# OPPO-Mente-Lab/X2I

Measured on AMD Instinct MI355X. Metric: images/sec, FLUX-schnell 1024x1024 4-step (projector + denoise loop), whole job, higher is better.
Workload: dtype bf16; 1 GPU; BASELINE configs[1]: qwen3b conditioning (C=37,H=2048,S_txt=512) -> projector -> shuttle-3/FLUX-schnell DiT 1024x1024, 4 steps; batch_per_gpu=4, global_batch=4, parallelism=batch-sharded x1, graph=True

## Files before the change

### x2i_amd/csrc/elementwise.hip

```cpp
#include "x2i_common.h"
#include "x2i_kernels.h"

namespace {

__device__ __forceinline__ void unpack8(const bf16x8_t& v, float (&f)[8]) {
#pragma unroll
  for (int i = 0; i < 8; ++i) f[i] = bf16_to_f32((bf16_t)v[i]);
}
__device__ __forceinline__ bf16x8_t pack8(const float (&f)[8]) {
  union { bf16x8_t v; uint32_t u[4]; } r;
#pragma unroll
  for (int i = 0; i < 4; ++i) r.u[i] = pack_bf16x2(f[2 * i], f[2 * i + 1]);
  return r.v;
}

constexpr int LN_MAXV = 8;

template <bool AFFINE>
__global__ __launch_bounds__(256) void ln_kernel(const bf16_t* __restrict__ X, long long x_bs, int ldx, bf16_t* __restrict__ Y,
                                                 long long y_bs, int ldy, int S, int D, int S0, const float* shift0,
                                                 const float* scale0, const float* shift1, const float* scale1,
                                                 long long mod_bs, const bf16_t* aw, const bf16_t* ab, float eps,
                                                 long long total_rows) {
  const int lane = threadIdx.x & 63;
// ... 193 lines not shown
                                                            int K, int act_in, int act_out, int accumulate, int rpw, long long x_gs, int rows_g) {
  typedef float f32x2 __attribute__((ext_vector_type(2)));
  if (blockIdx.y) {
    const long long g = blockIdx.y;
    Xv = (const char*)Xv + g * x_gs * (x_is_bf16 ? 2 : 4);
    W += g * N * K;
    if (bias) bias += g * N;
    Y += g * rows_g * ldy;
  }
  constexpr int NBP = NB == 1 ? 1 : (NB + 1) & ~1;
  extern __shared__ __attribute__((aligned(16))) float xs[];
  for (int i = threadIdx.x; i < NB * K; i += 256) {
    const int b = i / K, k = i - b * K;
    float v = x_is_bf16 ? bf16_to_f32(((const bf16_t*)Xv)[i]) : ((const float*)Xv)[i];
    xs[k * NBP + b] = apply_act(v, act_in);
  }
  __syncthreads();
  const int lane = threadIdx.x & 63;
  const int wave = threadIdx.x >> 6;
  const int n_base = (blockIdx.x * 4 + wave) * rpw;
  constexpr int R = 4;
  constexpr int NP = NB / 2;
#pragma unroll 1
  for (int rr = 0; rr < rpw; rr += R) {
    const int n0 = n_base + rr;
    if (n0 >= N) break;
    float acc[R][NB];
    f32x2 acc2[R][NP > 0 ? NP : 1];
#pragma unroll
    for (int r = 0; r < R; ++r) {
#pragma unroll
      for (int b = 0; b < NB; ++b) acc[r][b] = 0.f;
#pragma unroll
      for (int q = 0; q < NP; ++q) acc2[r][q] = f32x2{0.f, 0.f};
    }
    for (int k = lane * 8; k < K; k += 512) {
      bf16x8_t wv[R];
#pragma unroll
      for (int r = 0; r < R; ++r) {
        const int n = min(n0 + r, N - 1);
        wv[r] = __builtin_nontemporal_load((const bf16x8_t*)(W + (long long)n * K + k));
      }
      float wf[R][8];
#pragma unroll
      for (int r = 0; r < R; ++r) unpack8(wv[r], wf[r]);
#pragma unroll
      for (int j = 0; j < 8; ++j) {
        const float* xk = xs + (k + j) * NBP;
#pragma unroll
        for (int q = 0; q < NP; ++q) {
          const f32x2 x2 = *(const f32x2*)(xk + 2 * q);
#pragma unroll
          for (int r = 0; r < R; ++r) acc2[r][q] = __builtin_elementwise_fma(f32x2{wf[r][j], wf[r][j]}, x2, acc2[r][q]);
        }
        if constexpr (NB & 1) {
          const float x1 = xk[NB - 1];
#pragma unroll
          for (int r = 0; r < R; ++r) acc[r][NB - 1] = fmaf(wf[r][j], x1, acc[r][NB - 1]);
        }
      }
    }
#pragma unroll
    for (int r = 0; r < R; ++r)
#pragma unroll
      for (int q = 0; q < NP; ++q) { acc[r][2 * q] = acc2[r][q][0]; acc[r][2 * q + 1] = acc2[r][q][1]; }
#pragma unroll
    for (int r = 0; r < R; ++r) {
#pragma unroll
      for (int b = 0; b < NB; ++b) acc[r][b] = wave_sum(acc[r][b]);
      const int n = n0 + r;
      if (lane == 0 && n < N && rr + r < rpw) {
        const float bv = bias ? bf16_to_f32(bias[n]) : 0.f;
#pragma unroll
        for (int b = 0; b < NB; ++b) {
          float v = apply_act(acc[r][b] + bv, act_out);
          float* yp = Y + (long long)b * ldy + n;
          *yp = accumulate ? (*yp + v) : v;
        }
      }
    }
  }
}

__global__ void sinusoid_kernel(const float* __restrict__ t, float* __restrict__ out, int B, int dim, int round_bf16) {
  const int i = blockIdx.x * blockDim.x + threadIdx.x;
  const int half = dim / 2;
  if (i >= B * dim) return;
  const int b = i / dim, j = i - b * dim;
  const int k = j < half ? j : j - half;
  const float f = expf(-logf(10000.f) * (float)k / (float)half);
  const float a = t[b] * f;
  float v = j < half ? cosf(a) : sinf(a);
  if (round_bf16) v = bf16_to_f32(f32_to_bf16(v));
  out[i] = v;
}

__global__ void rope_table_kernel(const float* __restrict__ ids, int S, int d0, int d1, int d2, double theta, float* __restrict__ cosp,
                                  float* __restrict__ sinp) {
  const int D = d0 + d1 + d2;
  const long long i = (long long)blockIdx.x * blockDim.x + threadIdx.x;
  if (i >= (long long)S * D) return;
  const int s = (int)(i / D), c = (int)(i - (long long)s * D);
  int a = 0, start = 0, d = d0;
  if (c >= d0 + d1) a = 2, start = d0 + d1, d = d2;
  else if (c >= d0) a = 1, start = d0, d = d1;
  const int k = (c - start) >> 1;
  const double freq = 1.0 / pow(theta, (double)(2 * k) / (double)d);
  const double ang = (double)ids[(long long)s * 3 + a] * freq;
  cosp[i] = (float)cos(ang);
  sinp[i] = (float)sin(ang);
}

__global__ void euler_kernel(bf16_t* __restrict__ x, const bf16_t* __restrict__ eps, long long n8, const float* __restrict__ dt) {
  const float d = dt[0];
  for (long long i = (long long)blockIdx.x * blockDim.x + threadIdx.x; i < n8; i += (long long)gridDim.x * blockDim.x) {
    float a[8], e[8];
    unpack8(*(const bf16x8_t*)(x + i * 8), a);
    unpack8(*(const bf16x8_t*)(eps + i * 8), e);
#pragma unroll
    for (int j = 0; j < 8; ++j) a[j] = a[j] + d * e[j];
    *(bf16x8_t*)(x + i * 8) = pack8(a);
  }
}

__global__ __launch_bounds__(256) void gated_residual_kernel(bf16_t* __restrict__ X, long long x_bs, int ldx, const bf16_t* __restrict__ T,
                                                             long long t_bs, int ldt, const float* __restrict__ gate, long long g_bs, int S,
                                                             int D8, long long total) {
  for (long long i = (long long)blockIdx.x * blockDim.x + threadIdx.x; i < total; i += (long long)gridDim.x * blockDim.x) {
    const int c = (int)(i % D8);
    const long long row = i / D8;
    const int b = (int)(row / S), s = (int)(row - (long long)b * S);
    bf16_t* x = X + (long long)b * x_bs + (long long)s * ldx + c * 8;
    float a[8], t[8];
    unpack8(*(const bf16x8_t*)x, a);
    unpack8(*(const bf16x8_t*)(T + (long long)b * t_bs + (long long)s * ldt + c * 8), t);
    const float* g = gate + (long long)b * g_bs + c * 8;
#pragma unroll
    for (int j = 0; j < 8; ++j) a[j] = fmaf(g[j], t[j], a[j]);
    *(bf16x8_t*)x = pack8(a);
  }
}

__global__ void euler_tail_kernel(bf16_t* x, const bf16_t* eps, long long start, long long n, const float* dt) {
  const long long i = start + blockIdx.x * blockDim.x + threadIdx.x;
  if (i < n) x[i] = f32_to_bf16(bf16_to_f32(x[i]) + dt[0] * bf16_to_f32(eps[i]));
}

__global__ void cast_f32_bf16_kernel(const float* __restrict__ x, bf16_t* __restrict__ y, long long n) {
  for (long long i = (long long)blockIdx.x * blockDim.x + threadIdx.x; i < n; i += (long long)gridDim.x * blockDim.x)
    y[i] = f32_to_bf16(x[i]);
}
__global__ void cast_bf16_f32_kernel(const bf16_t* __restrict__ x, float* __restrict__ y, long long n) {
  for (long long i = (long long)blockIdx.x * blockDim.x + threadIdx.x; i < n; i += (long long)gridDim.x * blockDim.x)
    y[i] = bf16_to_f32(x[i]);
}

__global__ void seq_mean_kernel(const float* __restrict__ x, float* __restrict__ y, int S, int N) {
  const int n = blockIdx.x * blockDim.x + threadIdx.x, b = blockIdx.y;
  if (n >= N) return;
  const float* p = x + (long long)b * S * N + n;
  float acc = 0.f;
  for (int s = 0; s < S; ++s) acc += p[(long long)s * N];
  y[(long long)b * N + n] = acc / (float)S;
}

inline bool al16(const void* p) { return (((uintptr_t)p) & 15) == 0; }

}

int x2i_launch_ln_modulate(const void* X, long long x_bs, int ldx, void* Y, long long y_bs, int ldy, int B, int S, int D,
                           int S0, const float* shift0, const float* scale0, const float* shift1, const float* scale1,
                           long long mod_bs, float eps, hipStream_t stream) {
  if (!X || !Y || !shift1 || !scale1 || (S0 > 0 && (!shift0 || !scale0))) return x2i_set_error(X2I_ERR_ARG, "ln_modulate: null pointer");
  if (D % 8 || D > 64 * 8 * LN_MAXV || B <= 0 || S <= 0) return x2i_set_error(X2I_ERR_SHAPE, "ln_modulate: D=%d must be a multiple of 8 and <= %d", D, 64 * 8 * LN_MAXV);
  if (ldx % 8 || ldy % 8 || x_bs % 8 || y_bs % 8 || mod_bs % 4 || !al16(X) || !al16(Y)) return x2i_set_error(X2I_ERR_ALIGN, "ln_modulate: rows must be 16-byte aligned");
  const long long rows = (long long)B * S;
  if (D == 3072 && rows >= 4096) {
    hipLaunchKernelGGL((ln_rows_kernel<6, 4>), dim3((unsigned)((rows + 15) / 16)), dim3(256), 0, stream, (const bf16_t*)X, x_bs, ldx, (bf16_t*)Y, y_bs,
                       ldy, S, S0, shift0 ? shift0 : shift1, scale0 ? scale0 : scale1, shift1, scale1, mod_bs, eps, rows);
    return x2i_check_launch("ln_modulate");
  }
  hipLaunchKernelGGL(ln_kernel<false>, dim3((unsigned)((rows + 3) / 4)), dim3(256), 0, stream, (const bf16_t*)X, x_bs, ldx,
                     (bf16_t*)Y, y_bs, ldy, S, D, S0, shift0 ? shift0 : shift1, scale0 ? scale0 : scale1, shift1, scale1, mod_bs,
                     (const bf16_t*)nullptr, (const bf16_t*)nullptr, eps, rows);
  return x2i_check_launch("ln_modulate");
}

int x2i_launch_ln_affine(const void* X, void* Y, long long rows, int D, const void* w, const void* b, float eps, hipStream_t stream) {
  if (!X || !Y || !w || !b) return x2i_set_error(X2I_ERR_ARG, "ln_affine: null pointer");
  if (D % 8 || D > 64 * 8 * LN_MAXV || rows <= 0) return x2i_set_error(X2I_ERR_SHAPE, "ln_affine: D=%d unsupported", D);
  if (!al16(X) || !al16(Y) || !al16(w) || !al16(b)) return x2i_set_error(X2I_ERR_ALIGN, "ln_affine: 16-byte alignment required");
  hipLaunchKernelGGL(ln_kernel<true>, dim3((unsigned)((rows + 3) / 4)), dim3(256), 0, stream, (const bf16_t*)X, (long long)0, D,
                     (bf16_t*)Y, (long long)0, D, (int)1 << 30, D, 0, (const float*)nullptr, (const float*)nullptr,
                     (const float*)nullptr, (const float*)nullptr, (long long)0, (const bf16_t*)w, (const bf16_t*)b, eps, rows);
  return x2i_check_launch("ln_affine");
}

int x2i_launch_qkv_split(const void* qkv0, const void* qkv1, int ld0, int ld1, int B, int S, int S0, int H, const void* nq0,
                         const void* nk0, const void* nq1, const void* nk1, const float* cosp, const float* sinp, void* Q,
                         void* K, void* VT, int Spad, float eps, hipStream_t stream) {
  if (S0 < 0 || S0 > S || B <= 0 || S <= 0 || H <= 0) return x2i_set_error(X2I_ERR_SHAPE, "qkv_split: bad shape");
  if ((S0 > 0 && (!qkv0 || !nq0 || !nk0)) || (S0 < S && (!qkv1 || !nq1 || !nk1)) || !cosp || !sinp || !Q || !K || !VT)
    return x2i_set_error(X2I_ERR_ARG, "qkv_split: null pointer");
  if (Spad % 128 || Spad < S) return x2i_set_error(X2I_ERR_SHAPE, "qkv_split: Spad=%d must be a multiple of 128 and >= S=%d", Spad, S);
  if ((S0 > 0 && ld0 % 8) || (S0 < S && ld1 % 8)) return x2i_set_error(X2I_ERR_ALIGN, "qkv_split: ld must be a multiple of 8");
  hipLaunchKernelGGL(qk_norm_rope_kernel, dim3(S, B), dim3(256), 0, stream, (const bf16_t*)qkv0, (const bf16_t*)qkv1, ld0, ld1, S,
                     S0, H, (const bf16_t*)nq0, (const bf16_t*)nk0, (const bf16_t*)nq1, (const bf16_t*)nk1, cosp, sinp, (bf16_t*)Q,
                     (bf16_t*)K, Spad, eps);
  int rc = x2i_check_launch("qk_norm_rope");
  if (rc) return rc;
  hipLaunchKernelGGL(v_transpose_kernel, dim3((S + 63) / 64, H, B), dim3(256), 0, stream, (const bf16_t*)qkv0, (const bf16_t*)qkv1,
                     ld0, ld1, S, S0, H, (bf16_t*)VT, Spad);
  return x2i_check_launch("v_transpose");
}

int x2i_launch_skinny_linear(const void* X, int x_is_bf16, const void* W, const void* bias, float* Y, int ldy, int B, int N, int K,
                             int act_in, int act_out, int accumulate, hipStream_t stream) {
  return x2i_launch_skinny_linear_grouped(X, x_is_bf16, 0, W, bias, Y, ldy, 1, B, N, K, act_in, act_out, accumulate, stream);
}

int x2i_launch_skinny_linear_grouped(const void* X, int x_is_bf16, long long x_gs, const void* W, const void* bias, float* Y, int ldy, int G, int B,
                                     int N, int K, int act_in, int act_out, int accumulate, hipStream_t stream) {
  if (!X || !W || !Y) return x2i_set_error(X2I_ERR_ARG, "skinny_linear: null pointer");
  if (G <= 0 || G > 65535 || x_gs < 0) return x2i_set_error(X2I_ERR_SHAPE, "skinny_linear: bad group count / stride (G=%d)", G);
  if (G > 1 && B > SK_MAXB) return x2i_set_error(X2I_ERR_SHAPE, "skinny_linear_grouped: at most %d rows per group (B=%d)", SK_MAXB, B);
  if (B <= 0 || N <= 0 || K <= 0 || K % 8) return x2i_set_error(X2I_ERR_SHAPE, "skinny_linear: K=%d must be a multiple of 8", K);
  if (!al16(W)) return x2i_set_error(X2I_ERR_ALIGN, "skinny_linear: W must be 16-byte aligned");
  const int esz = x_is_bf16 ? 2 : 4;
  for (int b0 = 0; b0 < B; b0 += SK_MAXB) {
    const int nb = (B - b0) < SK_MAXB ? (B - b0) : SK_MAXB;
    const void* xp = (const char*)X + (long long)b0 * K * esz;
    float* yp = Y + (long long)b0 * ldy;
    const int rpw = N >= 65536 ? 16 : 4;
    const dim3 grid((N + 4 * rpw - 1) / (4 * rpw), G), block(256);
    const size_t shm = (size_t)(nb == 1 ? 1 : (nb + 1) & ~1) * K * 4;
    if (shm > 160 * 1024) return x2i_set_error(X2I_ERR_SHAPE, "skinny_linear: B*K too large for LDS");
#define SK_CASE(NB)                                                                                                   \
  case NB: {                                                                                                          \
    hipError_t e = hipFuncSetAttribute((const void*)skinny_linear_kernel<NB>, hipFuncAttributeMaxDynamicSharedMemorySize, \
                                       (int)shm);                                                                     \
    if (e != hipSuccess) return x2i_set_error(X2I_ERR_HIP, "skinny_linear: %s", hipGetErrorString(e));                \
    hipLaunchKernelGGL(skinny_linear_kernel<NB>, grid, block, shm, stream, xp, x_is_bf16, (const bf16_t*)W,           \
                       (const bf16_t*)bias, yp, ldy, N, K, act_in, act_out, accumulate, rpw, x_gs, B);               \
  } break;
    switch (nb) {
      SK_CASE(1) SK_CASE(2) SK_CASE(3) SK_CASE(4) SK_CASE(5) SK_CASE(6) SK_CASE(7) SK_CASE(8)
    }
#undef SK_CASE
    int rc = x2i_check_launch("skinny_linear");
    if (rc) return rc;
  }
  return X2I_OK;
}

int x2i_launch_timestep_sinusoid(const float* t, float* out, int B, int dim, int round_bf16, hipStream_t stream) {
  if (!t || !out || B <= 0 || dim <= 0 || dim % 2) return x2i_set_error(X2I_ERR_ARG, "timestep_sinusoid: bad argument");
  hipLaunchKernelGGL(sinusoid_kernel, dim3((B * dim + 255) / 256), dim3(256), 0, stream, t, out, B, dim, round_bf16);
  return x2i_check_launch("timestep_sinusoid");
}

int x2i_launch_rope_table(const float* ids, int S, int d0, int d1, int d2, float theta, float* cosp, float* sinp, hipStream_t stream) {
  if (!ids || !cosp || !sinp || S <= 0) return x2i_set_error(X2I_ERR_ARG, "rope_table: bad argument");
  if (d0 < 0 || d1 < 0 || d2 < 0 || (d0 | d1 | d2) & 1 || d0 + d1 + d2 <= 0 || theta <= 0.f)
    return x2i_set_error(X2I_ERR_SHAPE, "rope_table: axis dims must be even and non-negative (%d,%d,%d)", d0, d1, d2);
  const long long n = (long long)S * (d0 + d1 + d2);
  hipLaunchKernelGGL(rope_table_kernel, dim3((unsigned)((n + 255) / 256)), dim3(256), 0, stream, ids, S, d0, d1, d2, (double)theta, cosp, sinp);
  return x2i_check_launch("rope_table");
}

int x2i_launch_gated_residual(void* X, long long x_bs, int ldx, const void* T, long long t_bs, int ldt, const float* gate, long long g_bs,
                              int B, int S, int D, hipStream_t stream) {
  if (!X || !T || !gate || B <= 0 || S <= 0 || D <= 0) return x2i_set_error(X2I_ERR_ARG, "gated_residual: bad argument");
  if (D % 8 || ldx % 8 || ldt % 8 || x_bs % 8 || t_bs % 8 || g_bs % 4 || !al16(X) || !al16(T) || !al16(gate))
    return x2i_set_error(X2I_ERR_ALIGN, "gated_residual: rows must be 16-byte aligned, D %% 8 == 0");
  const long long total = (long long)B * S * (D / 8);
  const long long blocks = (total + 255) / 256;
  hipLaunchKernelGGL(gated_residual_kernel, dim3((unsigned)(blocks < 8192 ? blocks : 8192)), dim3(256), 0, stream, (bf16_t*)X, x_bs, ldx,
                     (const bf16_t*)T, t_bs, ldt, gate, g_bs, S, D / 8, total);
  return x2i_check_launch("gated_residual");
}

int x2i_launch_euler_step(void* x, const void* eps, long long n, const float* dt, hipStream_t stream) {
  if (!x || !eps || !dt || n <= 0) return x2i_set_error(X2I_ERR_ARG, "euler_step: bad argument");
  const long long n8 = (al16(x) && al16(eps)) ? n / 8 : 0;
  if (n8 > 0) {
    const long long blocks = (n8 + 255) / 256;
    hipLaunchKernelGGL(euler_kernel, dim3((unsigned)(blocks < 4096 ? blocks : 4096)), dim3(256), 0, stream, (bf16_t*)x,
                       (const bf16_t*)eps, n8, dt);
  }
  if (n8 * 8 < n) {
    const long long rem = n - n8 * 8;
    hipLaunchKernelGGL(euler_tail_kernel, dim3((unsigned)((rem + 255) / 256)), dim3(256), 0, stream, (bf16_t*)x, (const bf16_t*)eps,
                       n8 * 8, n, dt);
  }
  return x2i_check_launch("euler_step");
}

int x2i_launch_seq_mean(const float* x, float* y, int B, int S, int N, hipStream_t stream) {
  if (!x || !y || B <= 0 || S <= 0 || N <= 0) return x2i_set_error(X2I_ERR_ARG, "seq_mean: bad argument");
  hipLaunchKernelGGL(seq_mean_kernel, dim3((N + 255) / 256, B), dim3(256), 0, stream, x, y, S, N);
  return x2i_check_launch("seq_mean");
}

int x2i_launch_cast_f32_bf16(const float* x, void* y, long long n, hipStream_t stream) {
  if (!x || !y || n <= 0) return x2i_set_error(X2I_ERR_ARG, "cast: bad argument");
  const long long blocks = (n + 255) / 256;
  hipLaunchKernelGGL(cast_f32_bf16_kernel, dim3((unsigned)(blocks < 8192 ? blocks : 8192)), dim3(256), 0, stream, x, (bf16_t*)y, n);
  return x2i_check_launch("cast_f32_bf16");
}
int x2i_launch_cast_bf16_f32(const void* x, float* y, long long n, hipStream_t stream) {
  if (!x || !y || n <= 0) return x2i_set_error(X2I_ERR_ARG, "cast: bad argument");
  const long long blocks = (n + 255) / 256;
  hipLaunchKernelGGL(cast_bf16_f32_kernel, dim3((unsigned)(blocks < 8192 ? blocks : 8192)), dim3(256), 0, stream, (const bf16_t*)x, y, n);
  return x2i_check_launch("cast_bf16_f32");
}
```

### x2i_amd/flux.py

```python
import math
import os
from typing import Optional

import torch
import torch.nn as nn

from . import ops
from .ops import ACT_GELU_TANH, ACT_NONE, ACT_SILU


class _P(nn.Module):

    def __init__(self, **tensors):
        super().__init__()
        for k, v in tensors.items():
            self.register_parameter(k, nn.Parameter(v, requires_grad=False))


class _AttnTap(nn.Module):

    def forward(self, *outs):
        return outs if len(outs) > 1 else outs[0]


# ... 183 lines not shown
        self._ws = {}
        if getattr(self, "_fp8", None) is not None:
            self.enable_fp8(self._fp8_mode)
        return self

    @torch.no_grad()
    def init_random_(self, seed=0, std=0.02):
        gen = torch.Generator(device=self.device).manual_seed(seed)
        for k, t in self._fused.items():
            if k.endswith("norm_q") or k.endswith("norm_k") or k.endswith("norm_added_q") or k.endswith("norm_added_k"):
                t.copy_(1.0 + 0.1 * torch.randn(t.shape, device=t.device, generator=gen))
            else:
                flat = t.view(-1)
                step = 1 << 26
                for s in range(0, flat.numel(), step):
                    n = min(step, flat.numel() - s)
                    flat[s:s + n].copy_(std * torch.randn(n, device=t.device, generator=gen))
        return self

    def _workspace(self, B, St, Si):
        key = (B, St, Si)
        ws = self._ws.get(key)
        if ws is not None:
            return ws
        D, H = self.inner_dim, self._H
        S = St + Si
        Spad = ops.pad128(S)
        dev = self.device
        bf = dict(device=dev, dtype=torch.bfloat16)
        ws = dict(
            S=S, Spad=Spad,
            X=torch.empty((B, S, D), **bf), NRM=torch.empty((B, S, D), **bf), QKV=torch.empty((B * S, 3 * D), **bf),
            Q=torch.zeros((B, H, Spad, 128), **bf), K=torch.zeros((B, H, Spad, 128), **bf),
            VT=torch.zeros((B, H, 128, Spad), **bf), ATT=torch.empty((B, S, D), **bf),
            CAT=torch.empty((B * S, 5 * D), **bf), NRMF=torch.empty((B * Si, D), **bf),
            MOD=torch.empty((B, self._mod_rows), device=dev, dtype=torch.float32),
            TEMB=torch.empty((B, D), device=dev, dtype=torch.float32),
            H1=torch.empty((B, D), device=dev, dtype=torch.float32),
        )
        if self._fp8 is not None:
            f8 = dict(device=dev, dtype=ops.FP8)
            ws.update(NRM8=torch.empty((B, S, D), **f8), RS=torch.empty((B * S,), device=dev, dtype=torch.float32),
                      H8=torch.empty((B * Si, 4 * D), **f8), CAT8=torch.empty((B * S, 5 * D), **f8))
            if self._fp8_mode == "all":
                ws.update(ATT8=torch.empty((B, S, D), **f8))
        self._ws = {key: ws}
        return ws

    @torch.no_grad()
    def prepare_conditioning(self, encoder_hidden_states, pooled_projections, txt_ids, img_ids, guidance=None):
        cfg = self.config
        D = self.inner_dim
        enc = encoder_hidden_states
        B, St, Kj = enc.shape
        if txt_ids.ndim == 3:
            txt_ids = txt_ids[0]
        if img_ids.ndim == 3:
            img_ids = img_ids[0]
        Si = img_ids.shape[0]
        ws = self._workspace(B, St, Si)
        S = ws["S"]
        f = self._fused
        enc = enc.to(device=self.device, dtype=torch.bfloat16).contiguous()
        ctx = torch.empty((B, St, D), device=self.device, dtype=torch.bfloat16)
        ops.gemm(enc, f["context_embedder.w"], f["context_embedder.b"], out=ctx, M=B * St)
        ids = torch.cat((txt_ids.to(self.device), img_ids.to(self.device)), dim=0)
        cos, sin = ops.rope_table(ids, cfg.axes_dims_rope)
        pairs = ops.rope_pairs(cos, sin, check=False)
        cond = torch.empty((B, D), device=self.device, dtype=torch.float32)
        pooled = pooled_projections.to(device=self.device, dtype=torch.bfloat16).contiguous()
        h1 = ops.skinny_linear(pooled, f["tte.text_embedder.1.w"], f["tte.text_embedder.1.b"], out=ws["H1"], act_out=ACT_SILU)
        ops.skinny_linear(h1, f["tte.text_embedder.2.w"], f["tte.text_embedder.2.b"], out=cond)
        if cfg.guidance_embeds:
            if guidance is None:
                raise ValueError("guidance is required when config.guidance_embeds is True")
            g = (guidance.to(device=self.device, dtype=pooled_projections.dtype) * 1000).float().contiguous()
            gp = ops.timestep_sinusoid(g, 256, round_bf16=pooled_projections.dtype == torch.bfloat16)
            h1 = ops.skinny_linear(gp, f["tte.guidance_embedder.1.w"], f["tte.guidance_embedder.1.b"], out=ws["H1"], act_out=ACT_SILU)
            ops.skinny_linear(h1, f["tte.guidance_embedder.2.w"], f["tte.guidance_embedder.2.b"], out=cond, accumulate=True)
        return dict(B=B, St=St, Si=Si, ctx=ctx, cos=cos, sin=sin, rope_pairs=pairs, cond=cond, ws=ws,
                    round_bf16=pooled_projections.dtype == torch.bfloat16)

    MOD_GROUP = 4

    @torch.no_grad()
    def prepare_modulation(self, state, timesteps, dtype=torch.bfloat16):
        f = self._fused
        B, n = state["B"], len(timesteps)
        g = self.MOD_GROUP // B
        if g < 2:
            return [None] * n
        out = []
        for i0 in range(0, n, g):
            ts = timesteps[i0:i0 + g]
            t1000 = torch.cat([(t.to(device=self.device, dtype=dtype) * 1000).float().reshape(-1).expand(B) for t in ts]).contiguous()
            tp = ops.timestep_sinusoid(t1000, 256, round_bf16=state["round_bf16"])
            h1 = ops.skinny_linear(tp, f["tte.timestep_embedder.1.w"], f["tte.timestep_embedder.1.b"], act_out=ACT_SILU)
            temb = state["cond"].repeat(len(ts), 1)
            ops.skinny_linear(h1, f["tte.timestep_embedder.2.w"], f["tte.timestep_embedder.2.b"], out=temb, accumulate=True)
            table = ops.skinny_linear(temb, f["mod.w"], f["mod.b"], act_in=ACT_SILU)
            out += [table[k * B:(k + 1) * B] for k in range(len(ts))]
        return out

    @torch.no_grad()
    def denoise(self, state, hidden_states, timestep, control=None, mod=None):
        cfg = self.config
        f = self._fused
        ws = state["ws"]
        B, St, Si = state["B"], state["St"], state["Si"]
        S, Spad = ws["S"], ws["Spad"]
        D, H = self.inner_dim, self._H
        X, NRM, QKV, Q, K, VT, ATT, CAT, MOD = (ws[k] for k in ("X", "NRM", "QKV", "Q", "K", "VT", "ATT", "CAT", "MOD"))
        Ntot = self._mod_rows
        hs = hidden_states.to(device=self.device, dtype=torch.bfloat16).contiguous()
        X[:, :St].copy_(state["ctx"])
        ops.gemm(hs, f["x_embedder.w"], f["x_embedder.b"], out=X, M=Si, batch=B, a_batch_stride=Si * cfg.in_channels,
                 lda=cfg.in_channels, c_batch_stride=S * D, ldc=D, c_offset=St * D)
        t1000 = None
        if mod is None or control is not None:
            t1000 = (timestep.to(device=self.device, dtype=hidden_states.dtype) * 1000).float().contiguous()
        if mod is not None:
            MOD = mod
        else:
            tp = ops.timestep_sinusoid(t1000, 256, round_bf16=state["round_bf16"])
            h1 = ops.skinny_linear(tp, f["tte.timestep_embedder.1.w"], f["tte.timestep_embedder.1.b"], out=ws["H1"], act_out=ACT_SILU)
            temb = ws["TEMB"]
            temb.copy_(state["cond"])
            ops.skinny_linear(h1, f["tte.timestep_embedder.2.w"], f["tte.timestep_embedder.2.b"], out=temb, accumulate=True)
            ops.skinny_linear(temb, f["mod.w"], f["mod.b"], out=MOD, act_in=ACT_SILU)
        cos, sin = state["cos"], state["sin"]
        rc, rs = (state["rope_pairs"], None) if self.rope_pair_tables else (cos, sin)
        scale = 1.0 / math.sqrt(128.0)

        def mod(off):
            return MOD[:, off:]

        fuse_qkv = self.fuse_qkv and D % 64 == 0
        fp8 = self._fp8
        fp8_all = fp8 is not None and self._fp8_mode == "all"
        qs = scale * 1.4426950408889634 if (fuse_qkv or fp8_all) else 1.0
        scale = scale / qs if qs != 1.0 else scale
        vp_d = fuse_qkv and not fp8_all and ops.attention_prefers_vt_perm(H, S, scale)
        vp_s = fuse_qkv and fp8 is None and ops.attention_prefers_vt_perm(H, S, scale)
        taps = any(len(b.attn._forward_hooks) for b in self.transformer_blocks) or \
            any(len(b.attn._forward_hooks) for b in self.single_transformer_blocks)
        if taps and fp8 is not None:
            raise RuntimeError("attention taps (forward hooks on block.attn) are served by the bf16 configuration only")
        qkv_txt = QKV
        qkv_img_off = B * St * 3 * D
        for i in range(cfg.num_layers):
            p = f"d{i}"
            oi = i * 12 * D
            oc = oi + 6 * D
            if fp8_all:
                if St > 0:
                    ops.ln_modulate(X, NRM, B, St, D, St, mod(oc), mod(oc + D), mod(oc), mod(oc + D), Ntot, x_bs=S * D, y_bs=S * D)
                ops.ln_modulate_fp8(X, None, ws["NRM8"], ws["RS"], B, Si, D, 0, None, None, mod(oi), mod(oi + D), Ntot,
                                    x_bs=S * D, x_offset=St * D, y8_bs=S * D, y8_offset=St * D)
                wq, sq = fp8[p + ".qkv"]
                ops.gemm_qkv_fp8(ws["NRM8"], wq, f[p + ".qkv.b"], Q, K, VT, f[p + ".norm_q"], f[p + ".norm_k"], rc, rs, M=Si, H=H,
                                 Spad=Spad, tok_off=St, rows_per_sample=Si, batch=B, a_batch_stride=S * D, lda=D, a_offset=St * D,
                                 a_scale=ws["RS"], a_scale_batch_stride=Si, w_scale=sq, q_scale=qs)
                ops.gemm_qkv(NRM, f[p + ".cqkv.w"], f[p + ".cqkv.b"], Q, K, VT, f[p + ".norm_added_q"], f[p + ".norm_added_k"],
                             rc, rs, M=St, H=H, Spad=Spad, tok_off=0, rows_per_sample=St, batch=B, a_batch_stride=S * D, lda=D, q_scale=qs)
            else:
                ops.ln_modulate(X, NRM, B, S, D, St, mod(oc), mod(oc + D), mod(oi), mod(oi + D), Ntot)
            if fp8_all:
                pass
            elif fuse_qkv:
                g_img = dict(A=NRM, W=f[p + ".qkv.w"], bias=f[p + ".qkv.b"], Q=Q, K=K, VT=VT, norm_q=f[p + ".norm_q"], norm_k=f[p + ".norm_k"],
                             cos=rc, sin=rs, M=Si, H=H, Spad=Spad, tok_off=St, rows_per_sample=Si, batch=B, a_batch_stride=S * D, lda=D,
                             a_offset=St * D, q_scale=qs, vt_perm=vp_d)
                g_txt = dict(A=NRM, W=f[p + ".cqkv.w"], bias=f[p + ".cqkv.b"], Q=Q, K=K, VT=VT, norm_q=f[p + ".norm_added_q"],
                             norm_k=f[p + ".norm_added_k"], cos=rc, sin=rs, M=St, H=H, Spad=Spad, tok_off=0, rows_per_sample=St, batch=B,
                             a_batch_stride=S * D, lda=D, q_scale=qs, vt_perm=vp_d)
                if St > 0:
                    ops.gemm_qkv_pair(g_img, g_txt)
                else:
                    ops.gemm_qkv(**g_img)
            else:
                ops.gemm(NRM, f[p + ".qkv.w"], f[p + ".qkv.b"], out=QKV, M=Si, batch=B, a_batch_stride=S * D, lda=D,
                         a_offset=St * D, c_batch_stride=Si * 3 * D, ldc=3 * D, c_offset=qkv_img_off)
                ops.gemm(NRM, f[p + ".cqkv.w"], f[p + ".cqkv.b"], out=QKV, M=St, batch=B, a_batch_stride=S * D, lda=D,
                         c_batch_stride=St * 3 * D, ldc=3 * D)
                ops.qkv_split(qkv_txt, QKV.view(-1)[qkv_img_off:], 3 * D, 3 * D, B, S, St, H, f[p + ".norm_added_q"],
# ... 173 lines not shown
```

### x2i_amd/pipeline.py

```python
import math
from typing import Optional

import os

import numpy as np
import torch

from . import ops


class FlowMatchEulerDiscreteScheduler:

    def __init__(self, num_train_timesteps: int = 1000, shift: float = 1.0, use_dynamic_shifting: bool = False,
                 base_shift: float = 0.5, max_shift: float = 1.15, base_image_seq_len: int = 256,
                 max_image_seq_len: int = 4096):
        self.config = _Cfg(num_train_timesteps=num_train_timesteps, shift=shift, use_dynamic_shifting=use_dynamic_shifting,
                           base_shift=base_shift, max_shift=max_shift, base_image_seq_len=base_image_seq_len,
                           max_image_seq_len=max_image_seq_len)
        ts = np.linspace(1, num_train_timesteps, num_train_timesteps, dtype=np.float32)[::-1].copy()
        sig = ts / num_train_timesteps
        if not use_dynamic_shifting:
            sig = shift * sig / (1 + (shift - 1) * sig)
        self.sigma_min, self.sigma_max = float(sig[-1]), float(sig[0])
        self.timesteps = torch.from_numpy(sig * num_train_timesteps)
# ... 109 lines not shown
        latents = latents.view(batch_size, num_channels_latents, height // 2, 2, width // 2, 2)
        latents = latents.permute(0, 2, 4, 1, 3, 5)
        return latents.reshape(batch_size, (height // 2) * (width // 2), num_channels_latents * 4)

    @staticmethod
    def _unpack_latents(latents, height, width, vae_scale_factor):
        batch_size, num_patches, channels = latents.shape
        height = height // vae_scale_factor
        width = width // vae_scale_factor
        latents = latents.view(batch_size, height, width, channels // 4, 2, 2)
        latents = latents.permute(0, 3, 1, 4, 2, 5)
        return latents.reshape(batch_size, channels // (2 * 2), height * 2, width * 2)

    @staticmethod
    def _prepare_latent_image_ids(batch_size, height, width, device, dtype):
        ids = torch.zeros(height, width, 3)
        ids[..., 1] = ids[..., 1] + torch.arange(height)[:, None]
        ids[..., 2] = ids[..., 2] + torch.arange(width)[None, :]
        return ids.reshape(height * width, 3).to(device=device, dtype=dtype)

    def prepare_latents(self, batch_size, num_channels_latents, height, width, dtype, device, generator, latents=None):
        height = 2 * (int(height) // self.vae_scale_factor)
        width = 2 * (int(width) // self.vae_scale_factor)
        ids = self._prepare_latent_image_ids(batch_size, height // 2, width // 2, device, dtype)
        if latents is not None:
            return latents.to(device=device, dtype=dtype), ids
        shape = (batch_size, num_channels_latents, height, width)
        gdev = generator.device if generator is not None else device
        noise = torch.randn(shape, generator=generator, device=gdev, dtype=dtype).to(device)
        return self._pack_latents(noise, batch_size, num_channels_latents, height, width), ids

    @torch.no_grad()
    def __call__(self, prompt_embeds=None, pooled_prompt_embeds=None, num_inference_steps: int = 28,
                 guidance_scale: float = 3.5, height: Optional[int] = None, width: Optional[int] = None,
                 output_type: str = "latent", generator=None, latents=None, guided_hint=None, use_graph: bool = False,
                 return_dict: bool = True, **unused):
        if prompt_embeds is None or pooled_prompt_embeds is None:
            raise ValueError("x2i_amd FluxPipeline is driven by prompt_embeds/pooled_prompt_embeds (no text encoders), "
                             "as every reference inference script does")
        if output_type != "latent":
            raise ValueError('only output_type="latent" is on the hot path (VAE decode is the caller\'s, as in the reference)')
        tr = self.transformer
        ops.streamk_check(sync=False)
        height = height or self.default_sample_size * self.vae_scale_factor
        width = width or self.default_sample_size * self.vae_scale_factor
        if height % 16 or width % 16:
            raise ValueError("height and width must be multiples of 16")
        device = tr.device
        dtype = prompt_embeds.dtype
        B = prompt_embeds.shape[0]
        prompt_embeds = prompt_embeds.to(device)
        pooled_prompt_embeds = pooled_prompt_embeds.to(device)
        txt_ids = torch.zeros(prompt_embeds.shape[1], 3, device=device, dtype=dtype)
        C = tr.config.in_channels // 4
        latents, img_ids = self.prepare_latents(B, C, height, width, dtype, device, generator, latents)
        sc = self.scheduler.config
        sigmas = np.linspace(1.0, 1 / num_inference_steps, num_inference_steps)
        mu = calculate_shift(latents.shape[1], sc.base_image_seq_len, sc.max_image_seq_len, sc.base_shift, sc.max_shift)
        self.scheduler.set_timesteps(sigmas=sigmas, device=device, mu=mu)
        timesteps = self.scheduler.timesteps
        guidance = None
        if tr.config.guidance_embeds:
            guidance = torch.full([1], guidance_scale, device=device, dtype=torch.float32).expand(B)
        hint = guided_hint.to(device) if (self.control_nets is not None and guided_hint is not None) else None
        latents = latents.contiguous()
        if latents.dtype != torch.bfloat16:
            state = tr.prepare_conditioning(prompt_embeds, pooled_prompt_embeds, txt_ids, img_ids, guidance)
            control = self._control_fn(hint)
            for i, t in enumerate(timesteps):
                ts = t.expand(B).to(latents.dtype)
                noise = tr.denoise(state, latents, ts / 1000, control=control)
                latents = self.scheduler.step(noise.to(latents.dtype), t, latents)[0]
            return FluxPipelineOutput(latents) if return_dict else (latents,)

        dts = (self.scheduler.sigmas[1:] - self.scheduler.sigmas[:-1]).to(device=device, dtype=torch.float32).contiguous()
        tvals = [(t.expand(B).to(torch.bfloat16) / 1000).contiguous() for t in timesteps]

        aux = dict(txt_ids=txt_ids, img_ids=img_ids, guidance=guidance, dts=dts, tvals=tvals,
                   ws=tr._workspace(B, prompt_embeds.shape[1], latents.shape[1]))

        def body(pe, pooled, lat, hnt):
            state = tr.prepare_conditioning(pe, pooled, aux["txt_ids"], aux["img_ids"], aux["guidance"])
            control = self._control_fn(hnt)
            mods = tr.prepare_modulation(state, tvals, lat.dtype) if self.hoist_modulation else [None] * len(tvals)
            for i in range(len(tvals)):
                noise = tr.denoise(state, lat, tvals[i], control=control, mod=mods[i])
                ops.euler_step_(lat, noise, dts[i:i + 1])

        key = (B, prompt_embeds.shape[1], height, width, num_inference_steps, float(guidance_scale), hint is not None,
               getattr(self.transformer, "_fp8_mode", None),
               self.hoist_modulation,
               ops.option_epoch())
        entry = self._graphs.get(key) if use_graph else None
        if entry is None and not (use_graph and key in self._seen):
            latents = latents.clone()
            body(prompt_embeds, pooled_prompt_embeds, latents, hint)
            ops.streamk_poll()
            self.graph_stats["eager"] += 1
            self._seen[key] = True
            while len(self._seen) > 256:
                self._seen.pop(next(iter(self._seen)))
            return FluxPipelineOutput(latents) if return_dict else (latents,)
        if entry is None:
            torch.cuda.synchronize(device)
            torch.cuda.empty_cache()
            before = torch.cuda.memory_reserved(device)
            static = dict(pe=prompt_embeds.clone(), pooled=pooled_prompt_embeds.clone(), lat=latents.clone(),
                          hint=None if hint is None else hint.clone())
            aux["sk_ws"] = ops.StreamKWorkspace(device)
            graph = torch.cuda.CUDAGraph()
            with torch.cuda.graph(graph), ops.streamk_scope(aux["sk_ws"]):
                body(static["pe"], static["pooled"], static["lat"], static["hint"])
            torch.cuda.synchronize(device)
            nbytes = max(0, torch.cuda.memory_reserved(device) - before)
            entry = [graph, static, aux, nbytes]
            self._graphs[key] = entry
            self.graph_stats["captures"] += 1
            self._evict(keep=key)
        else:
            self._graphs[key] = self._graphs.pop(key)
        graph, static = entry[0], entry[1]
        static["pe"].copy_(prompt_embeds)
        static["pooled"].copy_(pooled_prompt_embeds)
        static["lat"].copy_(latents)
        if hint is not None:
            static["hint"].copy_(hint)
        graph.replay()
        entry[2]["sk_ws"].poll()
        self.graph_stats["replays"] += 1
        out = static["lat"].clone()
        return FluxPipelineOutput(out) if return_dict else (out,)

    def _evict(self, keep=None):
        def total():
            return sum(e[3] for e in self._graphs.values())
        while len(self._graphs) > 1 and (len(self._graphs) > self.graph_cache_entries or total() > self.graph_cache_bytes):
            victim = next(k for k in self._graphs if k != keep)
            del self._graphs[victim]
            self.graph_stats["evictions"] += 1

    def _control_fn(self, hint):
        if hint is None:
            return None
        from .lightcontrol import make_control_fn
        return make_control_fn(self.control_nets, hint)


class VaeImageProcessor:

    def __init__(self, vae_scale_factor: int = 8, do_normalize: bool = True):
        self.vae_scale_factor = vae_scale_factor
        self.do_normalize = do_normalize

    @staticmethod
    def denormalize(images):
        return (images / 2 + 0.5).clamp(0, 1)

    def postprocess(self, image, output_type: str = "pil"):
        image = image.detach().float()
        if self.do_normalize:
            image = self.denormalize(image)
        if output_type == "pt":
            return image
        arr = image.cpu().permute(0, 2, 3, 1).numpy()
        if output_type == "np":
            return arr
        if output_type != "pil":
# ... 8 lines not shown
```

Before: 4.538 images/s.

## Batch all-step modulation into one wide skinny GEMM with new kernel

```diff
diff --git a/x2i_amd/csrc/elementwise.hip b/x2i_amd/csrc/elementwise.hip
--- a/x2i_amd/csrc/elementwise.hip
+++ b/x2i_amd/csrc/elementwise.hip
@@ -299,6 +299,171 @@
   }
 }
 
+constexpr int SKW_MAXB = 16;
+constexpr int SKW_THREADS = 512;
+constexpr int SKW_R = 8;
+constexpr int SKW_TILE = (SKW_THREADS / 64) * SKW_R;
+constexpr int SKW_STEPS = 4;
+
+template <int NQ, bool XBF, int ACT>
+__device__ __forceinline__ void skw_stage(float* __restrict__ xs, const void* __restrict__ Xv, int nb, int K, int g0, int act_in) {
+  constexpr int U = NQ == 3 ? 3 : 4;
+  struct Raw { bf16x8_t h; f32x4_t lo, hi; };
+#pragma unroll 1
+  for (int m0 = 0; m0 < 2 * NQ; m0 += U) {
+    Raw raw[U];
+#pragma unroll
+    for (int u = 0; u < U; ++u) {
+      const int w = (m0 + u) * SKW_THREADS + threadIdx.x;
+      const int b = (w >> 10) * 4 + (w & 3), k = (g0 + ((w >> 8) & (SKW_STEPS - 1))) * 512 + ((w >> 2) & 63) * 8;
+      const long long off = (long long)min(b, nb - 1) * K + min(k, K - 8);
+      if constexpr (XBF) {
+        raw[u].h = *(const bf16x8_t*)((const bf16_t*)Xv + off);
+      } else {
+        raw[u].lo = *(const f32x4_t*)((const float*)Xv + off);
+        raw[u].hi = *(const f32x4_t*)((const float*)Xv + off + 4);
+      }
+    }
+#pragma unroll
+    for (int u = 0; u < U; ++u) {
+      const int w = (m0 + u) * SKW_THREADS + threadIdx.x;
+      const int b4 = w & 3, l = (w >> 2) & 63, il = (w >> 8) & (SKW_STEPS - 1), s = w >> 10;
+      const bool live = s * 4 + b4 < nb && (g0 + il) * 512 + l * 8 < K;
+      float v[8];
+      if constexpr (XBF) {
+        unpack8(raw[u].h, v);
+      } else {
+#pragma unroll
+        for (int j = 0; j < 4; ++j) { v[j] = raw[u].lo[j]; v[4 + j] = raw[u].hi[j]; }
+      }
+#pragma unroll
+      for (int j = 0; j < 8; ++j) {
+        if constexpr (ACT == 1) v[j] = silu_f(v[j]);
+        if constexpr (ACT == 2) v[j] = apply_act(v[j], act_in);
+        xs[(((il * 8 + j) * NQ + s) * 64 + l) * 4 + b4] = live ? v[j] : 0.f;
+      }
+    }
+  }
+}
+
+__device__ __forceinline__ float skw_sum64(float (&t)[64], int lane) {
+#pragma unroll
+  for (int o = 32; o > 0; o >>= 1) {
+    const bool hi = lane & o;
+#pragma unroll
+    for (int i = 0; i < o; ++i) {
+      const float x = t[2 * i], y = t[2 * i + 1];
+      t[i] = (hi ? y : x) + __shfl_xor(hi ? x : y, o, 64);
+    }
+  }
+  return t[0];
+}
+
+template <int NQ>
+__global__ __launch_bounds__(SKW_THREADS) void skinny_linear_wide_kernel(const void* __restrict__ Xv, int x_is_bf16, const bf16_t* __restrict__ W,
+                                                                         const bf16_t* __restrict__ bias, float* __restrict__ Y, int ldy, int nb,
+                                                                         int N, int K, int act_in, int act_out, int accumulate) {
+  typedef float f32x2 __attribute__((ext_vector_type(2)));
+  extern __shared__ __attribute__((aligned(16))) float xs[];
+  const int lane = threadIdx.x & 63;
+  const int wave = threadIdx.x >> 6;
+  const int ntiles = (N + SKW_TILE - 1) / SKW_TILE;
+  const int nsteps = (K + 511) >> 9;
+  constexpr int HR = SKW_R / 2;
+  const int mine_v = (int)(__brev((unsigned)lane) >> 26);
+  bf16x8_t wv[SKW_R];
+  int pt = blockIdx.x, pg = 0;
+  auto fetch_half = [&](int h) {
+    const int k = pg * 512 + lane * 8;
+    if (pt < ntiles && k < K) {
+      const int n0 = pt * SKW_TILE + wave * SKW_R + h * HR;
+#pragma unroll
+      for (int r = 0; r < HR; ++r) {
+        const int n = min(n0 + r, N - 1);
+        wv[h * HR + r] = __builtin_nontemporal_load((const bf16x8_t*)(W + (long long)n * K + k));
+      }
+    }
+    if (h == 1 && ++pg == nsteps) { pg = 0; pt += gridDim.x; }
+  };
+  fetch_half(0);
+  fetch_half(1);
+#pragma unroll 1
+  for (int tile = blockIdx.x; tile < ntiles; tile += gridDim.x) {
+    float bv[2];
+#pragma unroll
+    for (int h = 0; h < 2; ++h) {
+      const int n = tile * SKW_TILE + wave * SKW_R + h * HR + (mine_v >> 4);
+      bv[h] = bias && n < N ? bf16_to_f32(bias[n]) : 0.f;
+    }
+    f32x2 acc2[SKW_R][2 * NQ];
+#pragma unroll
+    for (int r = 0; r < SKW_R; ++r)
+#pragma unroll
+      for (int q = 0; q < 2 * NQ; ++q) acc2[r][q] = f32x2{0.f, 0.f};
+#pragma unroll 1
+    for (int g0 = 0; g0 < nsteps; g0 += SKW_STEPS) {
+      __syncthreads();
+      if (x_is_bf16) {
+        if (act_in == X2I_ACT_NONE) skw_stage<NQ, true, 0>(xs, Xv, nb, K, g0, act_in);
+        else if (act_in == X2I_ACT_SILU) skw_stage<NQ, true, 1>(xs, Xv, nb, K, g0, act_in);
+        else skw_stage<NQ, true, 2>(xs, Xv, nb, K, g0, act_in);
+      } else {
+        if (act_in == X2I_ACT_NONE) skw_stage<NQ, false, 0>(xs, Xv, nb, K, g0, act_in);
+        else if (act_in == X2I_ACT_SILU) skw_stage<NQ, false, 1>(xs, Xv, nb, K, g0, act_in);
+        else skw_stage<NQ, false, 2>(xs, Xv, nb, K, g0, act_in);
+      }
+      __syncthreads();
+#pragma unroll
+      for (int il = 0; il < SKW_STEPS; ++il) {
+        if (g0 + il < nsteps) {
+          const bool mine = (g0 + il) * 512 + lane * 8 < K;
+#pragma unroll
+          for (int h = 0; h < 2; ++h) {
+            if (mine) {
+              f32x4_t xq[2][NQ];
+#pragma unroll
+              for (int s = 0; s < NQ; ++s) xq[0][s] = *(const f32x4_t*)(xs + (((il * 8) * NQ + s) * 64 + lane) * 4);
+#pragma unroll
+              for (int j = 0; j < 8; ++j) {
+                if (j < 7) {
+#pragma unroll
+                  for (int s = 0; s < NQ; ++s) xq[(j + 1) & 1][s] = *(const f32x4_t*)(xs + (((il * 8 + j + 1) * NQ + s) * 64 + lane) * 4);
+                }
+#pragma unroll
+                for (int s = 0; s < NQ; ++s) {
+                  const f32x4_t x4 = xq[j & 1][s];
+                  const f32x2 xa = {x4[0], x4[1]}, xb = {x4[2], x4[3]};
+#pragma unroll
+                  for (int r = h * HR; r < h * HR + HR; ++r) {
+                    const float wf = bf16_to_f32((bf16_t)wv[r][j]);
+                    const f32x2 w2 = {wf, wf};
+                    acc2[r][2 * s] = __builtin_elementwise_fma(w2, xa, acc2[r][2 * s]);
+                    acc2[r][2 * s + 1] = __builtin_elementwise_fma(w2, xb, acc2[r][2 * s + 1]);
+                  }
+                }
+              }
+            }
+            fetch_half(h);
+          }
+        }
+      }
+    }
+#pragma unroll
+    for (int h = 0; h < 2; ++h) {
+      float t[64];
+#pragma unroll
+      for (int v = 0; v < 64; ++v) t[v] = (v & 15) < 4 * NQ ? acc2[h * HR + (v >> 4)][(v & 15) >> 1][v & 1] : 0.f;
+      const float sum = skw_sum64(t, lane);
+      const int n = tile * SKW_TILE + wave * SKW_R + h * HR + (mine_v >> 4), b = mine_v & 15;
+      if (b < nb && n < N) {
+        float v = apply_act(sum + bv[h], act_out);
+        float* yp = Y + (long long)b * ldy + n;
+        *yp = accumulate ? (*yp + v) : v;
+      }
+    }
+  }
+}
+
 __global__ void sinusoid_kernel(const float* __restrict__ t, float* __restrict__ out, int B, int dim, int round_bf16) {
   const int i = blockIdx.x * blockDim.x + threadIdx.x;
   const int half = dim / 2;
@@ -444,10 +609,30 @@
   if (B <= 0 || N <= 0 || K <= 0 || K % 8) return x2i_set_error(X2I_ERR_SHAPE, "skinny_linear: K=%d must be a multiple of 8", K);
   if (!al16(W)) return x2i_set_error(X2I_ERR_ALIGN, "skinny_linear: W must be 16-byte aligned");
   const int esz = x_is_bf16 ? 2 : 4;
-  for (int b0 = 0; b0 < B; b0 += SK_MAXB) {
-    const int nb = (B - b0) < SK_MAXB ? (B - b0) : SK_MAXB;
+  for (int b0 = 0; b0 < B;) {
     const void* xp = (const char*)X + (long long)b0 * K * esz;
     float* yp = Y + (long long)b0 * ldy;
+    if (G == 1 && B - b0 > SK_MAXB && al16(xp)) {
+      const int nb = (B - b0) < SKW_MAXB ? (B - b0) : SKW_MAXB;
+      const int nq = (nb + 3) / 4;
+      const int tiles = (N + SKW_TILE - 1) / SKW_TILE;
+      const dim3 grid(tiles < x2i_num_cus() ? tiles : x2i_num_cus()), block(SKW_THREADS);
+      const size_t shm = (size_t)nq * 4 * SKW_STEPS * 512 * 4;
+      const void* fn = nq == 3 ? (const void*)skinny_linear_wide_kernel<3> : (const void*)skinny_linear_wide_kernel<4>;
+      hipError_t e = hipFuncSetAttribute(fn, hipFuncAttributeMaxDynamicSharedMemorySize, (int)shm);
+      if (e != hipSuccess) return x2i_set_error(X2I_ERR_HIP, "skinny_linear: %s", hipGetErrorString(e));
+      if (nq == 3)
+        hipLaunchKernelGGL(skinny_linear_wide_kernel<3>, grid, block, shm, stream, xp, x_is_bf16, (const bf16_t*)W, (const bf16_t*)bias, yp,
+                           ldy, nb, N, K, act_in, act_out, accumulate);
+      else
+        hipLaunchKernelGGL(skinny_linear_wide_kernel<4>, grid, block, shm, stream, xp, x_is_bf16, (const bf16_t*)W, (const bf16_t*)bias, yp,
+                           ldy, nb, N, K, act_in, act_out, accumulate);
+      int rc = x2i_check_launch("skinny_linear_wide");
+      if (rc) return rc;
+      b0 += nb;
+      continue;
+    }
+    const int nb = (B - b0) < SK_MAXB ? (B - b0) : SK_MAXB;
     const int rpw = N >= 65536 ? 16 : 4;
     const dim3 grid((N + 4 * rpw - 1) / (4 * rpw), G), block(256);
     const size_t shm = (size_t)(nb == 1 ? 1 : (nb + 1) & ~1) * K * 4;
@@ -466,6 +651,7 @@
 #undef SK_CASE
     int rc = x2i_check_launch("skinny_linear");
     if (rc) return rc;
+    b0 += nb;
   }
   return X2I_OK;
 }
diff --git a/x2i_amd/flux.py b/x2i_amd/flux.py
--- a/x2i_amd/flux.py
+++ b/x2i_amd/flux.py
@@ -289,12 +289,15 @@
                     round_bf16=pooled_projections.dtype == torch.bfloat16)
 
     MOD_GROUP = 4
+    SCHEDULE_GROUP = 16
 
     @torch.no_grad()
     def prepare_modulation(self, state, timesteps, dtype=torch.bfloat16):
+        return self._modulation_tables(state, timesteps, dtype, self.MOD_GROUP // state["B"])
+
+    def _modulation_tables(self, state, timesteps, dtype, g):
         f = self._fused
         B, n = state["B"], len(timesteps)
-        g = self.MOD_GROUP // B
         if g < 2:
             return [None] * n
         out = []
@@ -308,6 +311,10 @@
             table = ops.skinny_linear(temb, f["mod.w"], f["mod.b"], act_in=ACT_SILU)
             out += [table[k * B:(k + 1) * B] for k in range(len(ts))]
         return out
+
+    @torch.no_grad()
+    def prepare_modulation_schedule(self, state, timesteps, dtype=torch.bfloat16):
+        return self._modulation_tables(state, timesteps, dtype, self.SCHEDULE_GROUP // state["B"])
 
     @torch.no_grad()
     def denoise(self, state, hidden_states, timestep, control=None, mod=None):
diff --git a/x2i_amd/pipeline.py b/x2i_amd/pipeline.py
--- a/x2i_amd/pipeline.py
+++ b/x2i_amd/pipeline.py
@@ -215,7 +215,12 @@
         def body(pe, pooled, lat, hnt):
             state = tr.prepare_conditioning(pe, pooled, aux["txt_ids"], aux["img_ids"], aux["guidance"])
             control = self._control_fn(hnt)
-            mods = tr.prepare_modulation(state, tvals, lat.dtype) if self.hoist_modulation else [None] * len(tvals)
+            if not self.hoist_modulation:
+                mods = [None] * len(tvals)
+            elif B > tr.MOD_GROUP // 2:
+                mods = tr.prepare_modulation_schedule(state, tvals, lat.dtype)
+            else:
+                mods = tr.prepare_modulation(state, tvals, lat.dtype)
             for i in range(len(tvals)):
                 noise = tr.denoise(state, lat, tvals[i], control=control, mod=mods[i])
                 ops.euler_step_(lat, noise, dts[i:i + 1])
```

Measured after the change: 4.554 images/s, median of 6. About the same (+0.4%).
